# Nexenta/edge-fuse

Hardware: NVIDIA H100
Metric: GiB/s hash+LZ4+dedup on 64 KiB chunks (higher is better)
Workload: dtype u8

## Files before the change

### edge_fuse_b200/csrc/lz4_encode.cuh

```cuda
#pragma once
#include "common.cuh"
#include "fingerprint.cuh"

namespace cmb {

constexpr uint32_t LZ4_MIN_MATCH = 4;
constexpr uint32_t LZ4_TAIL_LITERALS = 5;
constexpr uint32_t LZ4_MATCH_FIND_MARGIN = 12;
constexpr uint32_t LZ4_MIN_INPUT = 13;
constexpr uint32_t LZ4_NARROW_LIMIT = 65536 + 11;
constexpr uint32_t LZ4_FAR = 65535;
constexpr uint32_t LZ4_TABLE_BYTES = 16384;

__device__ __forceinline__ uint32_t lz4_hash4(uint32_t v) { return (v * 2654435761u) >> 19; }
__device__ __forceinline__ uint32_t lz4_hash5(uint64_t v) {
	return (uint32_t)(((v << 24) * 889523592379ULL) >> 52);
}

__device__ __forceinline__ uint32_t lz4_probe_off(uint32_t k, uint32_t accel) {
	if (k == 0) return 0;
	uint32_t m = k - 1, q = m >> 6, r = m & 63u;
	return 1u + accel * m + 32u * q * (q - 1u) + q * r;
}

template <bool WIDE> struct Lz4Table;
template <> struct Lz4Table<false> {
	uint16_t *t;
	__device__ __forceinline__ uint32_t get(uint32_t h) const { return t[h]; }
	__device__ __forceinline__ void put(uint32_t h, uint32_t pos) const { t[h] = (uint16_t)pos; }
};
template <> struct Lz4Table<true> {
	uint32_t *t;
	__device__ __forceinline__ uint32_t get(uint32_t h) const { return t[h]; }
	__device__ __forceinline__ void put(uint32_t h, uint32_t pos) const { t[h] = pos; }
};

struct Lz4Around { uint32_t before, at, next; };
__device__ __forceinline__ Lz4Around lz4_around(const uint8_t *src, uint32_t p) {
	const uint32_t a = p & ~3u, sh = (p & 3u) * 8u;
	const uint32_t *q = reinterpret_cast<const uint32_t *>(src + a);
	const uint32_t w0 = __ldg(q - (a != 0u));
	const uint32_t w1 = __ldg(q), w2 = __ldg(q + 1), w3 = __ldg(q + 2);
	Lz4Around r;
	r.before = __funnelshift_r(w0, w1, sh);
	r.at = __funnelshift_r(w1, w2, sh);
	r.next = __funnelshift_r(w2, w3, sh);
	return r;
}


__device__ __noinline__ uint32_t lz4_emit_len(uint8_t *dst, uint32_t op, uint32_t count, int lane) {
	uint32_t nff = count / 255u;
	for (uint32_t i = lane; i < nff; i += 32) dst[op + i] = 0xFF;
	if (lane == 0) dst[op + nff] = (uint8_t)(count - nff * 255u);
	return op + nff + 1;
}

__device__ __noinline__ void lz4_copy_literals(uint8_t *dst, const uint8_t *src, uint32_t len, int lane) {
	warp_copy_ro(dst, src, len, lane);
}

__device__ __noinline__ uint32_t lz4_count_long(const uint8_t *src, uint32_t a, uint32_t b, uint32_t lim,
    uint32_t lim4, int lane) {
	{
		const uint32_t pa = a + (uint32_t)lane;
		const bool same = pa < lim && ldg8(src + pa) == ldg8(src + b + (uint32_t)lane);
		const uint32_t stop = __ballot_sync(CMB_FULL, !same);
		if (stop) return (uint32_t)(__ffs(stop) - 1);
	}
	uint32_t total = 32;
	for (;;) {
		const uint32_t pa = a + total + 16u * lane;
		uint32_t nb = 0;
		if (pa < lim) {
			const uint32_t avail = min(16u, lim - pa);
			const uint32_t pb = b + total + 16u * lane;
#pragma unroll
			for (uint32_t j = 0; j < 4; j++) {
				if (nb == 4u * j && 4u * j < avail) {
					uint32_t x = read32u(src, pa + 4u * j, lim4) ^ read32u(src, pb + 4u * j, lim4);
					nb += x ? (uint32_t)(__ffs(x) - 1) >> 3 : 4u;
				}
			}
			nb = min(nb, avail);
		}
		const uint32_t stop = __ballot_sync(CMB_FULL, nb < 16u);
		if (stop) {
			int f = __ffs(stop) - 1;
			return total + 16u * f + __shfl_sync(CMB_FULL, nb, f);
		}
		total += 512u;
	}
}

__device__ __noinline__ uint32_t lz4_catchup_long(const uint8_t *src, uint32_t ip, uint32_t match,
    uint32_t anchor, int lane) {
	uint32_t total = 0;
	for (;;) {
		uint32_t k = total + lane + 1;
		bool ok = ip >= anchor + k && match >= k && ldg8(src + ip - k) == ldg8(src + match - k);
		uint32_t fail = __ballot_sync(CMB_FULL, !ok);
		if (fail) return total + (uint32_t)(__ffs(fail) - 1);
		total += 32;
	}
}

__device__ __forceinline__ uint64_t lz4_pack(bool found, bool retest, uint32_t ip, uint32_t match) {
	return ((uint64_t)found << 63) | ((uint64_t)retest << 62) | ((uint64_t)ip << 32) | match;
}

template <bool WIDE>
__device__ __noinline__ uint64_t lz4_search_slow(const uint8_t *src, uint32_t lim4, Lz4Table<WIDE> tab,
    uint32_t anchor, uint32_t shift, uint32_t accel, uint32_t mflimit, uint32_t g0, int lane, bool specials = true) {
	const uint32_t p0 = anchor + 1;
	for (;; g0 += 32) {
		const uint32_t g = g0 + lane;
		const bool special = g < shift;
		const uint32_t k = g - shift;
		uint32_t pos = p0 + lz4_probe_off(k, accel);
		const uint32_t nxt = p0 + lz4_probe_off(k + 1, accel);
		bool en = nxt <= mflimit;
		if (special) { pos = anchor - 2u + 2u * g; en = specials; }
		uint32_t h = 0x10000u + lane, pseq = 0, cand = 0;
		if (en) {
			if (WIDE) { uint64_t v = read64u(src, pos, lim4); pseq = (uint32_t)v; h = lz4_hash5(v); }
			else { pseq = read32u(src, pos, lim4); h = lz4_hash4(pseq); }
			cand = tab.get(h);
		}
		const uint32_t peers = __match_any_sync(CMB_FULL, h);
		const uint32_t lower = peers & ((1u << lane) - 1u);
		const uint32_t prev_pos = __shfl_sync(CMB_FULL, pos, lower ? 31 - __clz(lower) : lane);
		if (lower) cand = prev_pos;
		bool hit = false;
		if (en && !(special && g == 0) && cand + LZ4_FAR >= pos)
			hit = read32u(src, cand, lim4) == pseq;
		const uint32_t hits = __ballot_sync(CMB_FULL, hit);
		const uint32_t enmask = __ballot_sync(CMB_FULL, en);
		const int w = hits ? __ffs(hits) - 1 : 31;
		const uint32_t commit = hits ? (0xffffffffu >> (31 - w)) & enmask : enmask;
		if ((commit >> lane) & 1u) {
			const uint32_t pc = peers & commit;
			if (31 - __clz(pc) == lane) tab.put(h, pos);
		}
		__syncwarp();
		if (hits)
			return lz4_pack(true, g0 + (uint32_t)w < shift, __shfl_sync(CMB_FULL, pos, w),
			    __shfl_sync(CMB_FULL, cand, w));
		if (__ballot_sync(CMB_FULL, en || special) != CMB_FULL) return 0;
	}
}

__device__ __noinline__ uint32_t lz4_emit_general(uint8_t *dst, uint32_t op, const uint8_t *src, uint32_t anchor,
    uint32_t lit, uint32_t off, uint32_t mc, int lane) {
	if (lane == 0) dst[op] = (uint8_t)((min(lit, 15u) << 4) | min(mc, 15u));
	op++;
	if (lit >= 15u) op = lz4_emit_len(dst, op, lit - 15u, lane);
	if (lit <= 256u) {
		for (uint32_t i = lane; i < lit; i += 32) st_out8(dst + op + i, ldg8(src + anchor + i));
	} else {
		warp_copy_ro(dst + op, src + anchor, lit, lane);
	}
	op += lit;
	if (lane == 0) { dst[op] = (uint8_t)off; dst[op + 1] = (uint8_t)(off >> 8); }
	op += 2;
	if (mc >= 15u) op = lz4_emit_len(dst, op, mc - 15u, lane);
	return op;
}


}
```

### edge_fuse_b200/csrc/lz4_encode_ring.cuh

```cuda
#pragma once
#include "lz4_encode.cuh"
#include "kernels.h"

namespace cmb {

constexpr uint32_t RING_BYTES = 1024, RING_BUF = 256, RING_BUFS = 4;
constexpr uint32_t RING_MIRROR = 16;
constexpr uint32_t RING_ALLOC = RING_BYTES + 64;
constexpr uint32_t RING_AHEAD = 376;
constexpr uint32_t RING_MAX_ACCEL = 12;
constexpr uint32_t RING_MBAR_BYTES = 64;
constexpr uint32_t RING_WARP_SMEM = LZ4_TABLE_BYTES + RING_ALLOC + RING_MBAR_BYTES;

__device__ __forceinline__ uint32_t smem_addr(const void *p) { return (uint32_t)__cvta_generic_to_shared(p); }
__device__ __forceinline__ void mbar_init(uint32_t bar, uint32_t arrivals) {
	asm volatile("mbarrier.init.shared::cta.b64 [%0], %1;" ::"r"(bar), "r"(arrivals) : "memory");
}
__device__ __forceinline__ void mbar_expect_tx(uint32_t bar, uint32_t bytes) {
	asm volatile("mbarrier.arrive.expect_tx.shared::cta.b64 _, [%0], %1;" ::"r"(bar), "r"(bytes) : "memory");
}
__device__ __forceinline__ void tma_load_1d(uint32_t dst, const void *src, uint32_t bytes, uint32_t bar) {
	asm volatile("cp.async.bulk.shared::cluster.global.mbarrier::complete_tx::bytes [%0], [%1], %2, [%3];" ::"r"(dst),
	    "l"(src), "r"(bytes), "r"(bar)
	    : "memory");
}
__device__ __forceinline__ bool mbar_try_wait(uint32_t bar, uint32_t parity) {
	uint32_t ok;
	asm volatile("{\n\t.reg .pred p;\n\tmbarrier.try_wait.parity.shared::cta.b64 p, [%1], %2;\n\tselp.u32 %0, 1, 0, p;\n\t}"
	    : "=r"(ok)
	    : "r"(bar), "r"(parity)
	    : "memory");
	return ok != 0;
}

struct PageRing {
	const uint8_t *bytes;
	uint32_t s_bytes;
	uint32_t s_bar;
	uint32_t issued;
	uint32_t ready;
	uint32_t parity;
};

__device__ __forceinline__ void ring_wait_buf(uint32_t s_bar, uint32_t &parity, uint32_t g) {
	const uint32_t r = g & (RING_BUFS - 1u);
	while (!mbar_try_wait(s_bar + 8u * r, (parity >> r) & 1u)) {}
	parity ^= 1u << r;
}

__device__ __forceinline__ void ring_setup(PageRing &ring, uint8_t *ring_smem, uint8_t *bar_smem, int lane) {
	ring.bytes = ring_smem;
	ring.s_bytes = smem_addr(ring_smem);
	ring.s_bar = smem_addr(bar_smem);
	ring.issued = ring.ready = 0;
	ring.parity = 0;
	if (lane == 0) {
#pragma unroll
		for (uint32_t r = 0; r < RING_BUFS; r++) mbar_init(ring.s_bar + 8u * r, 1u);
		asm volatile("fence.mbarrier_init.release.cluster;" ::: "memory");
		asm volatile("fence.proxy.async.shared::cta;" ::: "memory");
	}
	__syncwarp();
}

__device__ __noinline__ uint64_t ring_advance(uint32_t s_bytes, uint32_t s_bar, uint64_t state, const uint8_t *src,
    uint32_t n, uint32_t nbufs, uint32_t g_lo, int lane) {
	uint32_t issued = (uint32_t)state & 0xffffu, ready = (uint32_t)(state >> 16) & 0xffffu, parity = (uint32_t)(state >> 32);
	const uint32_t g_hi = min(g_lo + 2u, nbufs - 1u);
	const uint32_t upto = min(issued, g_hi + 1u);
	while (ready < upto) { ring_wait_buf(s_bar, parity, ready); ready++; }
	if (issued < g_lo) { issued = g_lo; ready = g_lo; }
	const uint32_t want = min(g_lo + RING_BUFS, nbufs);
	__syncwarp();
	if (lane == 0) {
		for (uint32_t g = issued; g < want; g++) {
			const uint32_t r = g & (RING_BUFS - 1u);
			const uint32_t nb = min(RING_BUF, (n - g * RING_BUF + 15u) & ~15u);
			const uint8_t *from = src + (size_t)g * RING_BUF;
			mbar_expect_tx(s_bar + 8u * r, nb + (r == 0u ? RING_MIRROR : 0u));
			tma_load_1d(s_bytes + r * RING_BUF, from, nb, s_bar + 8u * r);
			if (r == 0u) tma_load_1d(s_bytes + RING_BYTES, from, RING_MIRROR, s_bar);
		}
	}
	if (issued < want) issued = want;
	while (ready <= g_hi) { ring_wait_buf(s_bar, parity, ready); ready++; }
	return (uint64_t)issued | ((uint64_t)ready << 16) | ((uint64_t)parity << 32);
}
__device__ __forceinline__ void ring_step(PageRing &ring, const uint8_t *src, uint32_t n, uint32_t nbufs, uint32_t g_lo,
    int lane) {
	const uint64_t st = ring_advance(ring.s_bytes, ring.s_bar,
	    (uint64_t)ring.issued | ((uint64_t)ring.ready << 16) | ((uint64_t)ring.parity << 32), src, n, nbufs, g_lo, lane);
	ring.issued = (uint32_t)st & 0xffffu; ring.ready = (uint32_t)(st >> 16) & 0xffffu; ring.parity = (uint32_t)(st >> 32);
}
__device__ __forceinline__ void ring_drain(PageRing &ring) {
	while (ring.ready < ring.issued) { ring_wait_buf(ring.s_bar, ring.parity, ring.ready); ring.ready++; }
}

__device__ __forceinline__ Lz4Around ring_around(const uint8_t *ring, uint32_t p) {
	const uint32_t sh = (p & 3u) * 8u;
	const uint32_t *q = reinterpret_cast<const uint32_t *>(ring + (((p & ~3u) - 4u) & (RING_BYTES - 1u)));
	const uint32_t w0 = q[0], w1 = q[1], w2 = q[2], w3 = q[3];
	Lz4Around r;
	r.before = __funnelshift_r(w0, w1, sh);
	r.at = __funnelshift_r(w1, w2, sh);
	r.next = __funnelshift_r(w2, w3, sh);
	return r;
}

template <bool WIDE, bool FP, bool RING>
__device__ uint32_t lz4_encode_lean(const uint8_t *__restrict__ src, uint32_t n, uint8_t *__restrict__ dst,
    uint32_t accel, uint8_t *tab_smem, PageRing &ring, int lane, uint64_t &fp_hi, uint64_t &fp_lo, uint32_t &ck) {
	Lz4Table<WIDE> tab;
	tab.t = reinterpret_cast<decltype(tab.t)>(tab_smem);
	const uint32_t lim4 = (n + 3u) & ~3u;
	uint32_t op = 0, anchor = 0;
	const uint32_t ck_span = n / CKPT_WORDS;
	uint32_t ck_k = 1, ck_at = ck_span ? ck_span : 0xffffffffu;
	ck = 0xffffffffu;
	EfFrontier fp;
	if (FP) fp.start(src, n, lane);

	{
		uint4 z = make_uint4(0, 0, 0, 0);
		uint4 *t4 = reinterpret_cast<uint4 *>(tab_smem);
#pragma unroll 4
		for (uint32_t i = lane; i < LZ4_TABLE_BYTES / 16; i += 32) t4[i] = z;
	}
	__syncwarp();

	if (n >= LZ4_MIN_INPUT) {
		const uint32_t mflimit = n - LZ4_MATCH_FIND_MARGIN;
		const uint32_t mlimit = n - LZ4_TAIL_LITERALS;
		const uint32_t nbufs = (n + RING_BUF - 1u) / RING_BUF;
		const uint8_t *const rb = ring.bytes;
		if (RING) ring.issued = ring.ready = 0;
		const bool special = lane < 2;
		const uint32_t kk = (uint32_t)lane - 2u;
		uint32_t delta2 = special ? 2u * (uint32_t)lane - 2u : 1u + (kk ? 1u + accel * (kk - 1u) : 0u);
		const uint32_t need2 = 2u + accel * kk;
		uint32_t en_below = special ? 0u : (mflimit >= need2 ? mflimit - need2 + 1u : 0u);
		const uint32_t special_on = special ? 0xffffffffu : 0u;
		asm volatile("" : "+r"(delta2), "+r"(en_below));
		bool started = false;
		constexpr uint32_t NARROW_W = 16u;
		constexpr int NARROW_HIT = 12;
		uint32_t width = 32u, calm = 0u;
		uint32_t next_event = 0, ring_next = 0;
		for (;;) {
			if (anchor >= next_event) {
				while (anchor >= ck_at) {
					const uint32_t rel = anchor - ck_at;
					if ((uint32_t)lane == ck_k) ck = rel < ck_span ? (op << CKPT_POS_BITS) | rel : 0xffffffffu;
					ck_k++;
					ck_at = ck_k < CKPT_WORDS ? ck_at + ck_span : 0xffffffffu;
				}
				if (anchor >= ring_next) {
				if (RING) {
					const uint32_t g_lo = (max(anchor, 4u) - 4u) / RING_BUF;
					if (ring.ready == g_lo + 2u && ring.issued == g_lo + 3u && g_lo + 3u < nbufs) {
						__syncwarp();
						if (lane == 0) {
							const uint32_t g = g_lo + 3u, r = g & (RING_BUFS - 1u);
							const uint32_t nb = min(RING_BUF, (n - g * RING_BUF + 15u) & ~15u);
							const uint8_t *from = src + (size_t)g * RING_BUF;
							mbar_expect_tx(ring.s_bar + 8u * r, nb + (r == 0u ? RING_MIRROR : 0u));
							tma_load_1d(ring.s_bytes + r * RING_BUF, from, nb, ring.s_bar + 8u * r);
							if (r == 0u) tma_load_1d(ring.s_bytes + RING_BYTES, from, RING_MIRROR, ring.s_bar);
						}
						ring.issued = g_lo + 4u;
						ring_wait_buf(ring.s_bar, ring.parity, g_lo + 2u);
						ring.ready = g_lo + 3u;
					} else {
						ring_step(ring, src, n, nbufs, g_lo, lane);
					}
					ring_next = (g_lo + 1u) * RING_BUF + 4u;
				} else {
					ring_next = (anchor | 255u) + 1u;
				}
				if (FP) fp.upto(src, anchor + 512u, lane);
				}
				next_event = min(ring_next, ck_at);
			}
			const bool en = anchor < en_below && (uint32_t)lane < width;
			const uint32_t pos = en ? anchor + delta2 : 0u;
			uint32_t litbyte, litbyte2;
			Lz4Around ai;
			if (RING) {
				litbyte = rb[(anchor + (uint32_t)lane) & (RING_BYTES - 1u)];
				litbyte2 = rb[(anchor + 32u + (uint32_t)lane) & (RING_BYTES - 1u)];
				ai = ring_around(rb, pos);
			} else {
				litbyte = ldg8(src + min(anchor + (uint32_t)lane, n - 1u));
				litbyte2 = ldg8(src + min(anchor + 32u + (uint32_t)lane, n - 1u));
				ai = lz4_around(src, pos);
			}

			const uint32_t pseq = ai.at;
			const uint32_t h = WIDE ? lz4_hash5((uint64_t)ai.at | ((uint64_t)ai.next << 32)) : lz4_hash4(ai.at);
			const uint32_t cand = tab.get(h);
			__syncwarp();
			if (en) tab.put(h, pos);
			__syncwarp();
			const Lz4Around ac = lz4_around(src, cand);
			const uint32_t seen = tab.get(h);
			__syncwarp();
			const bool foreign = en && seen != (WIDE ? pos : (pos & 0xffffu));
			bool hit = en && lane != 0 && ac.at == pseq;
			if (WIDE) hit = hit && cand + LZ4_FAR >= pos;
			const uint32_t foreigns = __ballot_sync(CMB_FULL, foreign);
			const uint32_t hits = __ballot_sync(CMB_FULL, hit);
			uint32_t nf, nb;
			{
				const uint32_t xf = ai.next ^ ac.next;
				nf = xf ? (uint32_t)(__ffs(xf) - 1) >> 3 : 4u;
				nf = min(nf, mlimit - min(pos + LZ4_MIN_MATCH, mlimit));
				const uint32_t xb = ai.before ^ ac.before;
				nb = xb ? (uint32_t)__clz(xb) >> 3 : 4u;
				nb = min(nb, min(pos - min(anchor, pos), cand));
				if (special) nb = 0;
			}
			const uint32_t low_hit = hits & (0u - hits), low_for = foreigns & (0u - foreigns);
			uint32_t ip, match, fwd, back;
			bool retest_hit;
			if (low_hit - 1u < low_for - 1u) {
				const int w = __ffs(hits) - 1;
				const uint32_t pos_w = __shfl_sync(CMB_FULL, pos, w);
				if (en && lane > w && !(foreign && seen <= (WIDE ? pos_w : (pos_w & 0xffffu)))) tab.put(h, cand);
				__syncwarp();
				ip = pos_w;
				match = __shfl_sync(CMB_FULL, cand, w);
				fwd = __shfl_sync(CMB_FULL, nf, w);
				back = __shfl_sync(CMB_FULL, nb, w);
				retest_hit = w == 1;
				calm = w < NARROW_HIT ? calm + 1u : 0u;
				if (w >= NARROW_HIT) width = 32u; else if (calm >= 8u) width = NARROW_W;
				if (fwd == 4u || back == 4u) {
					if (fwd == 4u) fwd = 4u + lz4_count_long(src, ip + 8u, match + 8u, mlimit, lim4, lane);
					if (back == 4u && ip >= anchor + 5u && match >= 5u)
						back = 4u + lz4_catchup_long(src, ip - 4u, match - 4u, anchor, lane);
				}
			} else {
				uint64_t res = 0;
				const uint32_t enmask = __ballot_sync(CMB_FULL, en || special || (uint32_t)lane >= width);
				const uint32_t w0 = width;
				width = 32u; calm = 0u;
				if (foreigns) {
					if (en) tab.put(h, cand);
					__syncwarp();
					res = lz4_search_slow<WIDE>(src, lim4, tab, anchor, 2u, accel, mflimit, 0, lane, started);
				} else if (enmask == CMB_FULL) {
					res = lz4_search_slow<WIDE>(src, lim4, tab, anchor, 2u, accel, mflimit, w0, lane, started);
				}
				if (!(res >> 63)) break;
				retest_hit = (res >> 62) & 1u;
				ip = (uint32_t)(res >> 32) & 0x3fffffffu;
				match = (uint32_t)res;
				fwd = lz4_count_long(src, ip + LZ4_MIN_MATCH, match + LZ4_MIN_MATCH, mlimit, lim4, lane);
				back = retest_hit ? 0u : lz4_catchup_long(src, ip, match, anchor, lane);
			}
			const uint32_t off = ip - match;
			const uint32_t mc = back + fwd;
			const uint32_t lit = ip - back - anchor;
			const uint32_t end = ip + LZ4_MIN_MATCH + fwd;

			if (lit <= 64u && mc < 15u + 255u) {
				uint8_t *o = dst + op;
				const uint32_t lext = lit >= 15u, mext = mc >= 15u;
				const uint32_t hl = 1u + lext;
				if ((uint32_t)lane < lit) st_out8(o + hl + lane, litbyte);
				if ((uint32_t)lane + 32u < lit) st_out8(o + hl + 32u + lane, litbyte2);
				const uint32_t tail = hl + lit;
				const uint32_t head4 = (min(lit, 15u) << 4) | min(mc, 15u) | (((lit - 15u) & 0xffu) << 8) | (off << 16);
				const uint32_t val = lane < 4 ? head4 >> (8u * (uint32_t)lane) : mc - 15u;
				const uint32_t at = lane < 2 ? (uint32_t)lane : tail + (uint32_t)lane - 2u;
				const uint32_t owners = 0x0du | (lext << 1) | (mext << 4);
				if ((owners >> lane) & 1u) st_out8(o + at, val);
				op += tail + 2u + mext;
			} else {
				op = lz4_emit_general(dst, op, src, anchor, lit, off, mc, lane);
			}

			anchor = end;
			started = true;
			en_below |= special_on;
			if (end > mflimit) break;
		}
		if (RING) ring_drain(ring);
	}

	while (ck_k < CKPT_WORDS && ck_span) {
		const uint32_t rel = anchor - ck_at;
		if ((uint32_t)lane == ck_k) ck = (anchor >= ck_at && rel < ck_span) ? (op << CKPT_POS_BITS) | rel : 0xffffffffu;
		ck_k++;
		ck_at += ck_span;
	}

	uint32_t run = n - anchor;
	if (lane == 0) dst[op] = (uint8_t)(min(run, 15u) << 4);
	op++;
	if (run >= 15u) op = lz4_emit_len(dst, op, run - 15u, lane);
	lz4_copy_literals(dst + op, src + anchor, run, lane);
	op += run;
	if (FP) fp.finish(src, n, lane, fp_hi, fp_lo);
	return op;
}

}
```

Measured before the change: 121.8.

## Defer LZ4 sequence emission to overlap with next iteration's candidate load latency

Each sequence's output is now written one iteration later. The emit is placed between issuing the candidate-word loads and consuming them, so store work can hide global-load latency. Literal bytes are captured after the deferred emit, and checkpoint offsets are adjusted to account for the pending sequence size. A predicated-store helper replaces branchy stores. This adds carried state and a final flush, which risks mistakes in the checkpoint and end-of-loop edge cases.

```diff
diff --git a/edge_fuse_b200/csrc/lz4_encode.cuh b/edge_fuse_b200/csrc/lz4_encode.cuh
--- a/edge_fuse_b200/csrc/lz4_encode.cuh
+++ b/edge_fuse_b200/csrc/lz4_encode.cuh
@@ -36,16 +36,25 @@
 };
 
 struct Lz4Around { uint32_t before, at, next; };
+struct Lz4Words { uint32_t w0, w1, w2, w3, sh; };
+__device__ __forceinline__ Lz4Words lz4_around_load(const uint8_t *src, uint32_t p) {
+	const uint32_t a = p & ~3u;
+	const uint32_t *q = reinterpret_cast<const uint32_t *>(src + a);
+	Lz4Words w;
+	w.w0 = __ldg(q - (a != 0u));
+	w.w1 = __ldg(q); w.w2 = __ldg(q + 1); w.w3 = __ldg(q + 2);
+	w.sh = (p & 3u) * 8u;
+	return w;
+}
+__device__ __forceinline__ Lz4Around lz4_around_align(const Lz4Words &w) {
+	Lz4Around r;
+	r.before = __funnelshift_r(w.w0, w.w1, w.sh);
+	r.at = __funnelshift_r(w.w1, w.w2, w.sh);
+	r.next = __funnelshift_r(w.w2, w.w3, w.sh);
+	return r;
+}
 __device__ __forceinline__ Lz4Around lz4_around(const uint8_t *src, uint32_t p) {
-	const uint32_t a = p & ~3u, sh = (p & 3u) * 8u;
-	const uint32_t *q = reinterpret_cast<const uint32_t *>(src + a);
-	const uint32_t w0 = __ldg(q - (a != 0u));
-	const uint32_t w1 = __ldg(q), w2 = __ldg(q + 1), w3 = __ldg(q + 2);
-	Lz4Around r;
-	r.before = __funnelshift_r(w0, w1, sh);
-	r.at = __funnelshift_r(w1, w2, sh);
-	r.next = __funnelshift_r(w2, w3, sh);
-	return r;
+	return lz4_around_align(lz4_around_load(src, p));
 }
 
 
@@ -54,6 +63,10 @@
 	for (uint32_t i = lane; i < nff; i += 32) dst[op + i] = 0xFF;
 	if (lane == 0) dst[op + nff] = (uint8_t)(count - nff * 255u);
 	return op + nff + 1;
+}
+__device__ __forceinline__ uint32_t lz4_len_bytes(uint32_t count) { return count >= 15u ? (count - 15u) / 255u + 1u : 0u; }
+__device__ __forceinline__ uint32_t lz4_seq_bytes(uint32_t lit, uint32_t mc) {
+	return 3u + lit + lz4_len_bytes(lit) + lz4_len_bytes(mc);
 }
 
 __device__ __noinline__ void lz4_copy_literals(uint8_t *dst, const uint8_t *src, uint32_t len, int lane) {
@@ -167,5 +180,30 @@
 	return op;
 }
 
-
-}
+__device__ __forceinline__ void st_out8_if(bool p, uint8_t *ptr, uint32_t v) {
+	asm volatile("{\n\t.reg .pred q;\n\tsetp.ne.u32 q, %2, 0;\n\t@q st.global.u8 [%0], %1;\n\t}" ::"l"(
+	                 __cvta_generic_to_global(ptr)), "r"(v), "r"((uint32_t)p)
+	             : "memory");
+}
+
+__device__ __forceinline__ void lz4_emit_seq(uint8_t *dst, const uint8_t *src, uint32_t op, uint32_t from, uint32_t lit,
+    uint32_t off, uint32_t mc, uint32_t b0, uint32_t b1, int lane) {
+	if (lit <= 64u && mc < 15u + 255u) {
+		uint8_t *o = dst + op;
+		const uint32_t lext = lit >= 15u, mext = mc >= 15u;
+		const uint32_t hl = 1u + lext;
+		st_out8_if((uint32_t)lane < lit, o + hl + lane, b0);
+		st_out8_if((uint32_t)lane + 32u < lit, o + hl + 32u + lane, b1);
+		const uint32_t tail = hl + lit;
+		const uint32_t head4 = (min(lit, 15u) << 4) | min(mc, 15u) | (((lit - 15u) & 0xffu) << 8) | (off << 16);
+		const uint32_t val = lane < 4 ? head4 >> (8u * (uint32_t)lane) : mc - 15u;
+		const uint32_t at = lane < 2 ? (uint32_t)lane : tail + (uint32_t)lane - 2u;
+		const uint32_t owners = 0x0du | (lext << 1) | (mext << 4);
+		st_out8_if((owners >> lane) & 1u, o + at, val);
+	} else {
+		lz4_emit_general(dst, op, src, from, lit, off, mc, lane);
+	}
+}
+
+
+}
diff --git a/edge_fuse_b200/csrc/lz4_encode_ring.cuh b/edge_fuse_b200/csrc/lz4_encode_ring.cuh
--- a/edge_fuse_b200/csrc/lz4_encode_ring.cuh
+++ b/edge_fuse_b200/csrc/lz4_encode_ring.cuh
@@ -146,11 +146,13 @@
 		constexpr int NARROW_HIT = 12;
 		uint32_t width = 32u, calm = 0u;
 		uint32_t next_event = 0, ring_next = 0;
+		uint32_t p_lit = 0, p_off = 0, p_mc = 0, litbyte = 0, litbyte2 = 0;
 		for (;;) {
 			if (anchor >= next_event) {
 				while (anchor >= ck_at) {
 					const uint32_t rel = anchor - ck_at;
-					if ((uint32_t)lane == ck_k) ck = rel < ck_span ? (op << CKPT_POS_BITS) | rel : 0xffffffffu;
+					const uint32_t at = op + (started ? lz4_seq_bytes(p_lit, p_mc) : 0u);
+					if ((uint32_t)lane == ck_k) ck = rel < ck_span ? (at << CKPT_POS_BITS) | rel : 0xffffffffu;
 					ck_k++;
 					ck_at = ck_k < CKPT_WORDS ? ck_at + ck_span : 0xffffffffu;
 				}
@@ -183,17 +185,7 @@
 			}
 			const bool en = anchor < en_below && (uint32_t)lane < width;
 			const uint32_t pos = en ? anchor + delta2 : 0u;
-			uint32_t litbyte, litbyte2;
-			Lz4Around ai;
-			if (RING) {
-				litbyte = rb[(anchor + (uint32_t)lane) & (RING_BYTES - 1u)];
-				litbyte2 = rb[(anchor + 32u + (uint32_t)lane) & (RING_BYTES - 1u)];
-				ai = ring_around(rb, pos);
-			} else {
-				litbyte = ldg8(src + min(anchor + (uint32_t)lane, n - 1u));
-				litbyte2 = ldg8(src + min(anchor + 32u + (uint32_t)lane, n - 1u));
-				ai = lz4_around(src, pos);
-			}
+			const Lz4Around ai = RING ? ring_around(rb, pos) : lz4_around(src, pos);
 
 			const uint32_t pseq = ai.at;
 			const uint32_t h = WIDE ? lz4_hash5((uint64_t)ai.at | ((uint64_t)ai.next << 32)) : lz4_hash4(ai.at);
@@ -201,9 +193,23 @@
 			__syncwarp();
 			if (en) tab.put(h, pos);
 			__syncwarp();
-			const Lz4Around ac = lz4_around(src, cand);
+			Lz4Words acw = lz4_around_load(src, cand);
 			const uint32_t seen = tab.get(h);
 			__syncwarp();
+
+			if (started) {
+				lz4_emit_seq(dst, src, op, anchor - LZ4_MIN_MATCH - p_mc - p_lit, p_lit, p_off, p_mc, litbyte, litbyte2, lane);
+				op += lz4_seq_bytes(p_lit, p_mc);
+			}
+			if (RING) {
+				litbyte = rb[(anchor + (uint32_t)lane) & (RING_BYTES - 1u)];
+				litbyte2 = rb[(anchor + 32u + (uint32_t)lane) & (RING_BYTES - 1u)];
+			} else {
+				litbyte = ldg8(src + min(anchor + (uint32_t)lane, n - 1u));
+				litbyte2 = ldg8(src + min(anchor + 32u + (uint32_t)lane, n - 1u));
+			}
+			asm volatile("" : "+r"(acw.w0), "+r"(acw.w1), "+r"(acw.w2), "+r"(acw.w3));
+			const Lz4Around ac = lz4_around_align(acw);
 			const bool foreign = en && seen != (WIDE ? pos : (pos & 0xffffu));
 			bool hit = en && lane != 0 && ac.at == pseq;
 			if (WIDE) hit = hit && cand + LZ4_FAR >= pos;
@@ -258,32 +264,19 @@
 				fwd = lz4_count_long(src, ip + LZ4_MIN_MATCH, match + LZ4_MIN_MATCH, mlimit, lim4, lane);
 				back = retest_hit ? 0u : lz4_catchup_long(src, ip, match, anchor, lane);
 			}
-			const uint32_t off = ip - match;
-			const uint32_t mc = back + fwd;
-			const uint32_t lit = ip - back - anchor;
+			p_off = ip - match;
+			p_mc = back + fwd;
+			p_lit = ip - back - anchor;
 			const uint32_t end = ip + LZ4_MIN_MATCH + fwd;
-
-			if (lit <= 64u && mc < 15u + 255u) {
-				uint8_t *o = dst + op;
-				const uint32_t lext = lit >= 15u, mext = mc >= 15u;
-				const uint32_t hl = 1u + lext;
-				if ((uint32_t)lane < lit) st_out8(o + hl + lane, litbyte);
-				if ((uint32_t)lane + 32u < lit) st_out8(o + hl + 32u + lane, litbyte2);
-				const uint32_t tail = hl + lit;
-				const uint32_t head4 = (min(lit, 15u) << 4) | min(mc, 15u) | (((lit - 15u) & 0xffu) << 8) | (off << 16);
-				const uint32_t val = lane < 4 ? head4 >> (8u * (uint32_t)lane) : mc - 15u;
-				const uint32_t at = lane < 2 ? (uint32_t)lane : tail + (uint32_t)lane - 2u;
-				const uint32_t owners = 0x0du | (lext << 1) | (mext << 4);
-				if ((owners >> lane) & 1u) st_out8(o + at, val);
-				op += tail + 2u + mext;
-			} else {
-				op = lz4_emit_general(dst, op, src, anchor, lit, off, mc, lane);
-			}
 
 			anchor = end;
 			started = true;
 			en_below |= special_on;
 			if (end > mflimit) break;
+		}
+		if (started && anchor > mflimit) {
+			lz4_emit_seq(dst, src, op, anchor - LZ4_MIN_MATCH - p_mc - p_lit, p_lit, p_off, p_mc, litbyte, litbyte2, lane);
+			op += lz4_seq_bytes(p_lit, p_mc);
 		}
 		if (RING) ring_drain(ring);
 	}
```

Measured after the change: 131.6 (median of 6 runs). 8.0% higher.
